# alebal123bal/BayesOpt_smart

Measured on AMD Instinct MI355X. Metric: candidate-points/sec (GP predict + HVI) at N_train=512, N_cand=1M, higher is better.
Workload: dtype f64; 1 GPU; C3: 2D/2-obj toy_function, N_train=512, N_cand=1,048,576 per GPU ('ij' integer grid), HVI (Sigma-UCB), q=3; n_train=512, n_cand_per_gpu=1048576, n_cand_total=1048576, n_objectives=2, dim=2, topq=3, parallelism=candidate-shard x1, step_launch=hip_graph, candidate_offset=0

## Files before the change

bayesopt_smart_amd/csrc/bo_gridconv.hip:

```cpp

#include "bo_predict_impl.h"

namespace {

using namespace bo;

constexpr int kListWaves = 4;
constexpr int kListChunk = 512;
#ifndef BO_ACC_RB
#define BO_ACC_RB 8
#endif
constexpr int kAccRB = BO_ACC_RB;
constexpr int kAccRows = 64 * kAccRB;
constexpr int kAccUnroll = 4;
constexpr int kClassLists = kConvClasses * kConvShards;
static_assert(kClassLists % 64 == 0 && kClassLists <= 2 * 64 * kConvAccWaves &&
              (kConvShards & (kConvShards - 1)) == 0 && kConvShards <= 16 && kConvShards <= kConvCountStride,
              "conv_acc_kernel's scan and lookup of the class lists");
#ifndef BO_CONV_PF
#define BO_CONV_PF 3
#endif
constexpr int kConvPF = BO_CONV_PF;
constexpr int kContractWaves = 8;
constexpr size_t kConvLdsBytes = 160 * 1024;
constexpr double kPairDrop = 0x1p-100;
constexpr double kTabFlush = 0x1p-128;

struct ListLds {
  int order, rc, nm;
  size_t bytes;
  __host__ __device__ ListLds(int n, int C)
      : order(C + 1), rc(order + n), nm(rc + 2 * n), bytes((size_t)(nm + kListWaves * kListChunk) * sizeof(int)) {}
};
struct AccLds {
  int ints, part;
  size_t bytes;
  __host__ __device__ explicit AccLds(int R)
      : ints(4 * R), part(kClassLists + 1),
        bytes((size_t)ints * sizeof(double) + (size_t)(part + kConvAccWaves + 1) / 2 * 2 * sizeof(int)) {}
};
struct ContractLds {
  int HB, tabH, hband, cn;
  size_t bytes;
  __host__ __device__ ContractLds(int C, int Cpad, int LT, int NP, int lists = 0)
      : HB(Cpad + LT / 2), tabH(2 * HB), hband(tabH + Cpad + C - 1), cn(hband + 1),
        bytes((size_t)cn * sizeof(double) + (size_t)NP * sizeof(int)) {
    if (bytes < (size_t)lists * sizeof(TopEntry)) bytes = (size_t)lists * sizeof(TopEntry);
  }
};

__device__ __forceinline__ void conv_list_done(const ConvArgs& a, int tau, int kept, int lane, int dyn) {
  if (kept == 0) {
    for (int o = 0; o < a.n_obj; ++o) {
      double* row = a.T + ((size_t)o * a.LT + tau) * a.ldr;
      for (int i = lane; i < a.ldr; i += 64) row[i] = 0.0;
    }
  }
  if (lane == 0) {
    a.pkept[tau] = kept;
    if (dyn && kept > 0) {
      const int e = 31 - __clz(kept);
      const int cls = 2 * e + (e > 0 ? (kept >> (e - 1)) & 1 : 0);
      const int sh = tau & (kConvShards - 1);
      const int slot = atomicAdd(a.ccount + cls * kConvCountStride + sh, 1);
      a.clist[(size_t)(cls * kConvShards + sh) * (a.LT / kConvShards) + slot] = tau;
    }
  }
}

__global__ __launch_bounds__(64 * kListWaves) void conv_list_kernel(const ConvArgs a, int tau_blocks, int dyn) {
  if (__builtin_amdgcn_readfirstlane(*a.flag) != 0) return;
  const int tid = threadIdx.x;
  if ((int)blockIdx.x >= tau_blocks) {
    const long long total = (long long)a.NP * a.ldr;
    const long long stride = (long long)(gridDim.x - tau_blocks) * (64 * kListWaves);
    for (int o = 0; o < a.n_obj; ++o) {
      const double nhl = a.nhl[o], pv = a.pv[o];
      double* tm = a.Tm + (size_t)o * a.NP * a.ldr;
      for (long long t = (long long)(blockIdx.x - tau_blocks) * (64 * kListWaves) + tid; t < total; t += stride) {
        const int s = (int)(t / a.ldr), i = (int)(t - (long long)s * a.ldr);
        double v = 0.0;
        if (s < a.n && i < a.nrows) {
          const int n = a.order[s];
          const double d = (double)(a.row_lo + i - a.rc[2 * n]);
          v = pv * a.alpha[(size_t)o * a.n_pad + n] * exp(nhl * (d * d));
        }
        tm[t] = v;
      }
    }
    return;
  }
  extern __shared__ __attribute__((aligned(16))) int si[];
  const ListLds L(a.n, a.C);
  int* cstart = si;
  int* order = si + L.order;
  int* rc = si + L.rc;
  for (int t = tid; t <= a.C; t += 64 * kListWaves) cstart[t] = a.cstart[t];
  for (int t = tid; t < a.n; t += 64 * kListWaves) order[t] = a.order[t];
  for (int t = tid; t < 2 * a.n; t += 64 * kListWaves) rc[t] = a.rc[t];
  __syncthreads();
  const int lane = tid & 63, wave = tid >> 6;
  int* nm = si + L.nm + wave * kListChunk;
  const int tau = blockIdx.x * kListWaves + wave;
  if (tau >= a.LT) return;
  int s0 = 0, s1 = 0;
  for (int c = lane; c < a.C; c += 64) {
    const int h = cstart[c + 1] - cstart[c];
    const int x0 = tau - c, x1 = x0 + 1;
    s0 += h * cstart[x0 < 0 ? 0 : x0 > a.C ? a.C : x0];
    s1 += h * cstart[x1 < 0 ? 0 : x1 > a.C ? a.C : x1];
  }
#pragma unroll
  for (int d = 32; d > 0; d >>= 1) {
    s0 += __shfl_xor(s0, d, 64);
    s1 += __shfl_xor(s1, d, 64);
  }
  const int h0 = (tau + 1) >> 1, h1 = (tau + 2) >> 1;
  const int p0 = __builtin_amdgcn_readfirstlane((s0 + cstart[h0 > a.C ? a.C : h0]) >> 1);
  const int total = __builtin_amdgcn_readfirstlane((s1 + cstart[h1 > a.C ? a.C : h1]) >> 1) - p0;
  if (lane == 0) a.pstart[tau] = p0;
  if (total == 0) {
    conv_list_done(a, tau, 0, lane, dyn);
    return;
  }
  const int R2 = 2 * a.R;
  const int per = (a.n + 63) / 64;
  const int n_lo = lane * per < a.n ? lane * per : a.n;
  const int n_hi = n_lo + per < a.n ? n_lo + per : a.n;
  int mine = 0;
  for (int n = n_lo; n < n_hi; ++n) {
    const int pc = tau - rc[2 * n + 1];
    if (pc < 0 || pc >= a.C) continue;
    for (int s = cstart[pc]; s < cstart[pc + 1]; ++s) mine += order[s] >= n ? 1 : 0;
  }
  int incl = mine;
#pragma unroll
  for (int d = 1; d < 64; d <<= 1) {
    const int v = __shfl_up(incl, d, 64);
    if (lane >= d) incl += v;
  }
  const int first = incl - mine;
  int kept = 0;
  for (int cb = 0; cb < total; cb += kListChunk) {
    const int cnt = total - cb < kListChunk ? total - cb : kListChunk;
    if (first < cb + cnt && first + mine > cb) {
// ... 69 lines not shown
    const double* e = tb + s;
#pragma unroll
    for (int k = 0; k < kAccRB; ++k) ev[k] = e[it[k]];
  };
  auto term = [&](double wv, const double (&ev)[kAccRB]) {
#pragma unroll
    for (int k = 0; k < kAccRB; ++k) {
      const double t = __dmul_rn(wv, ev[k]);
      const double te = __builtin_fma(wv, ev[k], -t);
      const double s2 = __dadd_rn(hi[k], t);
      const double bb = __dsub_rn(s2, hi[k]);
      const double se = __dadd_rn(__dsub_rn(hi[k], __dsub_rn(s2, bb)), __dsub_rn(t, bb));
      hi[k] = s2;
      lo[k] = __dadd_rn(lo[k], __dadd_rn(se, te));
    }
  };
  int p = 0;
  for (; p + kAccUnroll <= cnt; p += kAccUnroll) {
    double wv[kAccUnroll];
    int sv[kAccUnroll];
#pragma unroll
    for (int u = 0; u < kAccUnroll; ++u) {
      wv[u] = w[p + u];
      sv[u] = sl[p + u];
    }
    double ev[2][kAccRB];
    gather(sv[0], ev[0]);
#pragma unroll
    for (int u = 0; u < kAccUnroll; ++u) {
      if (u + 1 < kAccUnroll) gather(sv[u + 1], ev[(u + 1) & 1]);
      term(wv[u], ev[u & 1]);
    }
  }
  for (; p < cnt; ++p) {
    double ev[kAccRB];
    gather(sl[p], ev);
    term(w[p], ev);
  }
#pragma unroll
  for (int k = 0; k < kAccRB; ++k) {
    const int i = ib + lane + 64 * k;
    if (FULL) Trow[i] = hi[k] + lo[k];
    else if (i < ldr) Trow[i] = i < nrows ? hi[k] + lo[k] : 0.0;
  }
}

__global__ __launch_bounds__(64 * kConvAccWaves) void conv_acc_kernel(
    const ConvArgs a, const double* __restrict__ pair_w, const int* __restrict__ pair_sl,
    const int* __restrict__ pstart, const int* __restrict__ pkept, const int* __restrict__ ccount,
    const int* __restrict__ clist, int* __restrict__ ticket, double* __restrict__ T, int nrb, int ngrp, int dyn) {
  if (__builtin_amdgcn_readfirstlane(*a.flag) != 0) return;
  extern __shared__ __attribute__((aligned(16))) double sd[];
  const int tid = threadIdx.x, lane = tid & 63, o = blockIdx.y;
  const double nhl = a.nhl[o];
  const int R2 = 2 * a.R;
  const AccLds L(a.R);
  double* tabE = sd;
  int* cst = (int*)(sd + L.ints);
  int* part = cst + L.part;
  for (int t = tid; t < 2 * R2; t += 64 * kConvAccWaves) {
    const int par = t >= R2 ? 1 : 0, h = t - par * R2;
    const double m = (double)(2 * h + par - (R2 - 2));
    tabE[t] = exp(0.5 * nhl * (m * m));
  }
  if (dyn) {
    int c[2], sum = 0;
#pragma unroll
    for (int u = 0; u < 2; ++u) {
      const int j = 2 * tid + u;
      c[u] = j < kClassLists ? ccount[(kConvClasses - 1 - j / kConvShards) * kConvCountStride + j % kConvShards] : 0;
      sum += c[u];
    }
    int incl = sum;
#pragma unroll
    for (int d = 1; d < 64; d <<= 1) {
      const int v = __shfl_up(incl, d, 64);
      if (lane >= d) incl += v;
    }
    if (lane == 63) part[tid >> 6] = incl;
    __syncthreads();
    int run = incl - sum;
    for (int w = 0; w < (tid >> 6); ++w) run += part[w];
#pragma unroll
    for (int u = 0; u < 2; ++u) {
      const int j = 2 * tid + u;
      if (j < kClassLists) cst[j] = run;
      run += c[u];
      if (j == kClassLists - 1) cst[kClassLists] = run;
    }
  }
  __syncthreads();
  const int n_items = (dyn ? cst[kClassLists] : a.LT) * nrb;
  const double* wo = pair_w + (size_t)o * a.n_pairs;
  const int g = blockIdx.x % ngrp;
  int* tk = ticket + (o * kConvTicketGroups + g) * kConvTicketStride;
  for (int k = (blockIdx.x / ngrp) * kConvAccWaves + (tid >> 6);;) {
    const int t = k * ngrp + g;
    if (t >= n_items) break;
    int nx = 0;
    if (dyn && lane == 0) nx = atomicAdd(tk, 1);
    const int oi = t / nrb, rb = t - oi * nrb;
    int tau = oi;
    if (dyn) {
      constexpr int per = kClassLists / 64;
      const unsigned long long b1 = __ballot(cst[per * lane + per] > oi);
      const int l1 = __builtin_ctzll(b1);
      const unsigned long long b2 = __ballot(cst[per * l1 + (lane < per ? lane : per - 1) + 1] > oi);
      const int j = per * l1 + __builtin_ctzll(b2);
      const int cls = kConvClasses - 1 - j / kConvShards;
      const int* list = clist + (size_t)(cls * kConvShards + j % kConvShards) * (a.LT / kConvShards);
      tau = __builtin_amdgcn_readfirstlane(list[oi - cst[j]]);
    }
    const int p0 = __builtin_amdgcn_readfirstlane(pstart[tau]);
    const int cnt = __builtin_amdgcn_readfirstlane(pkept[tau]);
    if (!dyn && cnt == 0) break;
    const int ib = rb * kAccRows;
    double* Trow = T + ((size_t)o * a.LT + tau) * a.ldr;
// ... 17 lines not shown

template <int NB, class BGen>
__device__ __forceinline__ void conv_gemm(const double* __restrict__ X, int ldr, int nkb, int g, d4 (&acc)[NB],
                                          BGen&& bgen) {
  double ring[kConvPF][4];
#pragma unroll
  for (int p = 0; p < kConvPF; ++p) conv_load_a(X, ldr, p < nkb ? p : nkb - 1, g, ring[p]);
  for (int kb0 = 0; kb0 < nkb; kb0 += kConvPF) {
#pragma unroll
    for (int p = 0; p < kConvPF; ++p) {
      const int kb = kb0 + p;
      if (kb < nkb) {
        double av[4];
#pragma unroll
        for (int s = 0; s < 4; ++s) av[s] = ring[p][s];
        const int nx = kb + kConvPF;
        conv_load_a(X, ldr, nx < nkb ? nx : nkb - 1, g, ring[p]);
        double bv[4][NB];
        bgen(kb, bv);
#pragma unroll
        for (int s = 0; s < 4; ++s)
#pragma unroll
          for (int nb = 0; nb < NB; ++nb) acc[nb] = mfma64(av[s], bv[s][nb], acc[nb]);
      }
    }
  }
}

template <int NB>
__global__ __launch_bounds__(64 * kContractWaves) void conv_contract_kernel(const ConvArgs a) {
  if (__builtin_amdgcn_readfirstlane(*a.flag) != 0) return;
  extern __shared__ __attribute__((aligned(16))) double sd[];
  const ContractLds L(a.C, a.Cpad, a.LT, a.NP);
  double* tabB = sd;
  double* tabH = sd + L.tabH;
  int* hband = (int*)(sd + L.hband);
  int* cn = (int*)(sd + L.cn);
  constexpr int TW = 16 * NB;
  const int tid = threadIdx.x, lane = tid & 63, wave = tid >> 6;
  const int nt = blockDim.x, W = nt >> 6;
  const int g = lane >> 4, jl = lane & 15;
  const int cb_n = a.Cpad / TW;
  const long long n_wt = (long long)(a.ldr / 16) * cb_n;
  const long long gi_lo = a.cand_offset, gi_hi = a.cand_offset + a.n_cand;
#ifndef BO_ABL_CT_NOOUT
  const bool outs = true;
#else
  const bool outs = a.ld_out < 0;
#endif
  for (int t = tid; t < a.NP; t += nt) cn[t] = t < a.n ? a.rc[2 * a.order[t] + 1] : 0;

  double lv = -__builtin_inf();
  long long li = -1;
  double tab_nhl = __builtin_nan("");
  for (long long base = (long long)blockIdx.x * W; base < n_wt; base += (long long)gridDim.x * W) {
    const long long wt = base + wave;
    const bool active = wt < n_wt;
    const long long wtc = active ? wt : n_wt - 1;
    const int i0 = (int)(wtc / cb_n) * 16, j0 = (int)(wtc % cb_n) * TW;
    double acq[NB][4];
    for (int o = 0; o < a.n_obj; ++o) {
      const double nhl = a.nhl[o];
      if (!(nhl == tab_nhl)) {
        __syncthreads();
        int mq = 0;
        int mm = 0;
#ifndef BO_ABL_CT_NOTAB
        for (int t = tid; t < 2 * L.HB; t += nt) {
          const int par = t >= L.HB ? 1 : 0, h = t - par * L.HB;
          const int mi = 2 * h + par - (a.LT - 1);
          const double m = (double)mi;
          const double v = exp(0.5 * nhl * (m * m));
          const bool flush = v < kTabFlush;
          tabB[t] = flush ? 0.0 : v;
          if (!flush) mq = max(mq, abs(mi));
        }
        for (int t = tid; t < a.Cpad + a.C - 1; t += nt) {
          const int mi = t - (a.C - 1);
          const double m = (double)mi;
          const double v = exp(nhl * (m * m));
          const bool flush = v < kTabFlush;
          tabH[t] = flush ? 0.0 : v;
          if (!flush) mm = max(mm, abs(mi));
        }
#else
        mm = min((int)sqrt(128.0 * 0.6931471805599453 / -nhl), a.C - 1);
        mq = min((int)sqrt(256.0 * 0.6931471805599453 / -nhl), a.LT - 1);
#endif
        if (tid < 2) hband[tid] = 0;
        __syncthreads();
#pragma unroll
        for (int d = 32; d > 0; d >>= 1) {
          mq = max(mq, __shfl_xor(mq, d, 64));
          mm = max(mm, __shfl_xor(mm, d, 64));
        }
        if (lane == 0) {
          atomicMax(hband, mq);
          atomicMax(hband + 1, mm);
        }
        __syncthreads();
        tab_nhl = nhl;
      }
      int kq_lo = 0, kq_hi = a.LT / 16;
      if (!a.full) {
        const int hq = hband[0];
        const int t_hi = 2 * (j0 + TW - 1) + hq < a.LT - 1 ? 2 * (j0 + TW - 1) + hq : a.LT - 1;
        const int t_lo = 2 * j0 - hq > 0 ? (2 * j0 - hq < t_hi ? 2 * j0 - hq : t_hi) : 0;
        kq_lo = __builtin_amdgcn_readfirstlane(t_lo >> 4);
        kq_hi = __builtin_amdgcn_readfirstlane((t_hi >> 4) + 1);
      }
      d4 aq[NB], am[NB];
#pragma unroll
      for (int nb = 0; nb < NB; ++nb) {
        aq[nb] = (d4){0.0, 0.0, 0.0, 0.0};
        am[nb] = (d4){0.0, 0.0, 0.0, 0.0};
      }
      const double* Tq = a.T + ((size_t)o * a.LT + 16 * kq_lo) * a.ldr + i0 + jl;
      int km_lo = 0, km_hi = a.NP / 16;
      if (!a.full) {
        const int hm = hband[1];
        const int c_hi = j0 + TW + hm < a.C ? j0 + TW + hm : a.C;
        const int c_lo = j0 - hm > 0 ? (j0 - hm < a.C ? j0 - hm : a.C) : 0;
        km_lo = __builtin_amdgcn_readfirstlane(a.cstart[c_lo] >> 4);
        km_hi = __builtin_amdgcn_readfirstlane((a.cstart[c_hi] + 15) >> 4);
      }
      const double* Tm = a.Tm + ((size_t)o * a.NP + 16 * km_lo) * a.ldr + i0 + jl;
      const double* pe0 = tabB + (a.LT / 2 - 1 - 8 * kq_lo - 2 * g) + j0 + jl;
#ifdef BO_ABL_CT_BCONST
      const double bconst = pe0[0];
#endif
      conv_gemm<NB>(Tq, a.ldr, kq_hi - kq_lo, g, aq, [&](int kb, double (&bv)[4][NB]) {
#ifdef BO_ABL_CT_BCONST
#pragma unroll
        for (int s = 0; s < 4; ++s)
#pragma unroll
          for (int nb = 0; nb < NB; ++nb) bv[s][nb] = bconst;
#else
        const double* pe = pe0 - 8 * kb;
        const double* po = pe + L.HB;
#pragma unroll
        for (int nb = 0; nb < NB; ++nb) {
          bv[0][nb] = po[16 * nb];
          bv[1][nb] = pe[16 * nb];
          bv[2][nb] = po[16 * nb - 1];
          bv[3][nb] = pe[16 * nb - 1];
        }
#endif
      });
      const int* cn0 = cn + 16 * km_lo + 4 * g;
      if (km_hi > km_lo) conv_gemm<NB>(Tm, a.ldr, km_hi - km_lo, g, am, [&](int kb, double (&bv)[4][NB]) {
#ifdef BO_ABL_CT_BCONST
#pragma unroll
        for (int s = 0; s < 4; ++s)
#pragma unroll
// ... 161 lines not shown
      const long long e0 = (long long)gridDim.x * q, e1 = (long long)a.n_lists * q;
      for (long long e = e0 + tid; e < e1; e += nt) {
        a.partial[e].v = -__builtin_inf();
        a.partial[e].i = -1;
      }
    }
  }
}

}

namespace bo {

bool conv_lds_admits(int n, int R, int C, int Cpad, int LT, int NP) {
  const size_t bound = ((size_t)4 * R + 2048) * sizeof(double) + ((size_t)(C + 1) + 3 * (size_t)n + 2048) * sizeof(int);
  assert(ConvSetupLds(n, C, 256).bytes <= bound && ListLds(n, C).bytes <= bound && AccLds(R).bytes <= bound);
  return bound <= kConvLdsBytes && ContractLds(C, Cpad, LT, NP).bytes <= kConvLdsBytes;
}

template <class K>
static hipError_t conv_lds_attr(K k, size_t lds) {
  if (lds <= 64 * 1024) return hipSuccess;
  return hipFuncSetAttribute((const void*)k, hipFuncAttributeMaxDynamicSharedMemorySize, (int)lds);
}

ConvSched conv_acc_schedule(int R, int LT, int ldr, int n_obj, int cus) {
  ConvSched sc;
  sc.nrb = (ldr + kAccRows - 1) / kAccRows;
  const long long items = (long long)LT * sc.nrb;
  const size_t tab = (size_t)4 * R * sizeof(double);
  const int per_cu = (int)(kConvLdsBytes / tab < 4 ? kConvLdsBytes / tab : 4);
  long long wgs = (long long)(cus > 0 ? cus : 256) * per_cu / n_obj;
  if (wgs > (items + kConvAccWaves - 1) / kConvAccWaves) wgs = (items + kConvAccWaves - 1) / kConvAccWaves;
  if (wgs < 1) wgs = 1;
  sc.wgs = (int)wgs;
  sc.ngrp = (int)(wgs < kConvTicketGroups ? wgs : kConvTicketGroups);
  sc.dyn = (items <= wgs * kConvAccWaves && wgs % sc.ngrp == 0) ? 0 : 1;
  return sc;
}

hipError_t launch_gridconv(const ConvArgs& ca, const ConvPlan& cp, const ConvSched& sc, hipStream_t st) {
  const size_t l1 = ListLds(ca.n, ca.C).bytes, la = AccLds(ca.R).bytes;
  const size_t l2 = ContractLds(ca.C, ca.Cpad, ca.LT, ca.NP, cp.waves * ca.topq).bytes;
  if (l1 > kConvLdsBytes || la > kConvLdsBytes) return hipErrorInvalidValue;
  if (cp.waves < 1 || cp.waves > kContractWaves || cp.grid > ca.n_lists) return hipErrorInvalidValue;
  auto* contract = cp.nb == 4 ? conv_contract_kernel<4> : cp.nb == 2 ? conv_contract_kernel<2> : conv_contract_kernel<1>;
  hipError_t e;
  if ((e = conv_lds_attr(conv_list_kernel, l1)) != hipSuccess) return e;
  if ((e = conv_lds_attr(conv_acc_kernel, la)) != hipSuccess) return e;
  if ((e = conv_lds_attr(contract, l2)) != hipSuccess) return e;
  const int tau_blocks = (ca.LT + kListWaves - 1) / kListWaves;
  const long long tm_elems = (long long)ca.NP * ca.ldr;
  const int tm_blocks = (int)((tm_elems + 1023) / 1024 < 512 ? (tm_elems + 1023) / 1024 : 512);
  hipLaunchKernelGGL(conv_list_kernel, dim3(tau_blocks + tm_blocks), dim3(64 * kListWaves), l1, st, ca, tau_blocks,
                     sc.dyn);
  if ((e = hipGetLastError()) != hipSuccess) return e;
  hipLaunchKernelGGL(conv_acc_kernel, dim3((unsigned)sc.wgs, ca.n_obj), dim3(64 * kConvAccWaves), la, st, ca,
                     (const double*)ca.pair_w, (const int*)ca.pair_sl, (const int*)ca.pstart, (const int*)ca.pkept,
                     (const int*)ca.ccount, (const int*)ca.clist, ca.ticket, ca.T, sc.nrb, sc.ngrp, sc.dyn);
  if ((e = hipGetLastError()) != hipSuccess) return e;
  hipLaunchKernelGGL(contract, dim3(cp.grid), dim3(64 * cp.waves), l2, st, ca);
  return hipGetLastError();
}

}
```

bayesopt_smart_amd/csrc/bo_predict.hip:

```cpp

#include "bo_predict_impl.h"

#include <vector>

namespace {

__device__ __forceinline__ double kstar_at(const FusedArgs& a, int o, int f, long long j, bool valid) {
  return (valid && f < a.n_train) ? a.kstar[((long long)o * a.ks_rows + f) * a.n_cand + j] : 0.0;
}

template <int NS, bool SELECT>
__device__ __forceinline__ void contract_epair(__amdgpu_buffer_rsrc_t wr, int voff, int base,
                                               int& pos, int ep, const double (&B)[NS],
                                               d2 (&wa)[kPF], d2 (&wb)[kPF], d4& acc0, d4& acc1,
                                               double (&sel0)[4], double (&sel1)[4]) {
  constexpr int NCH = NS / 8;
#pragma unroll
  for (int c = 0; c < NCH; ++c) {
#pragma unroll
    for (int pp = 0; pp < 4; ++pp) {
      const int p = 4 * c + pp;
      const d2 ca = wa[pp];
      const d2 cb = wb[pp];
      const int so = base + ((pos + kPF) << 11);
// ... 400 lines not shown
  return cus;
}

constexpr double kConvMargin = 1.15;
constexpr int kConvMaxN = 4096;

void plan_gridconv(const bo_predict_desc* d, Plan* pl, bool kmem, int cus) {
  if (kmem || !pl->cm || d->cand_kind != BO_CAND_GRID || d->dim != 2 || d->n_cand <= 0) return;
  if (d->mode & (BO_PREDICT_DENSE | BO_PREDICT_NO_SEPARABLE | BO_PREDICT_FP32 | BO_PREDICT_NO_GRID_CONV)) return;
  const char* env = getenv("BO_GRID_CONV");
  if (env && env[0] == '0' && env[1] == 0) return;
  const long long R = d->grid_shape[0], C = d->grid_shape[1], n = d->n_train;
  if (R < 1 || C < 1 || R > (1 << 15) || C > (1 << 15) || n > kConvMaxN) return;
  if (d->cand_offset < 0 || d->cand_offset + d->n_cand > R * C) return;
  bo::ConvPlan cp = {};
  cp.row_lo = (int)(d->cand_offset / C);
  cp.nrows = (int)((d->cand_offset + d->n_cand - 1) / C) - cp.row_lo + 1;
  cp.ldr = (cp.nrows + 15) / 16 * 16;
  cp.Cpad = (int)((C + 63) / 64 * 64);
  cp.LT = (int)((2 * C - 1 + 15) / 16 * 16);
  cp.NP = (int)((n + 15) / 16 * 16);
  if (!bo::conv_lds_admits((int)n, (int)R, (int)C, cp.Cpad, cp.LT, cp.NP)) return;
  const long long wave_tiles = (long long)(cp.ldr / 16) * (cp.Cpad / 64);
  if (!(d->mode & (BO_PREDICT_GRID_CONV | BO_PREDICT_GRID_CONV_FULL))) {
    const double nch = pl->n_pad / 32;
    const double F = (double)d->n_obj * 1024.0 * nch * (nch + 1);
    const double old_rounds = (double)(((d->n_cand + 63) / 64 + 255) / 256);
    const double old_us = 25.0 + old_rounds * 64.0 * (F / 273.0e3 + 0.038);
    const double pairs_per_tau = 0.5 * (double)n * (double)(n + 1) / (double)(2 * C - 1);
    const double pair_us = 2.2 * pairs_per_tau * (double)((cp.ldr + 1023) / 1024) *
                           (double)((d->n_obj * (2 * C - 1) + 4095) / 4096);
    const double tile_rounds = (double)((wave_tiles + 1023) / 1024);
    const double contract_us = tile_rounds * 2048.0 * (double)(cp.LT + cp.NP) * (double)d->n_obj / 48.8e3;
    const double conv_us = 60.0 + pair_us + contract_us;
    if (!(kConvMargin * conv_us < old_us)) return;
  }
  cp.planned = true;
  const long long tiles64 = wave_tiles;
  cp.nb = tiles64 >= 8LL * cus ? 4 : 2 * tiles64 >= 8LL * cus ? 2 : 1;
  const char* tile = getenv("BO_CONV_TILE");
  if (tile && (tile[0] == '1' || tile[0] == '2' || tile[0] == '4') && tile[1] == 0) cp.nb = tile[0] - '0';
  const long long tiles = tiles64 * (4 / cp.nb);
  cp.waves = tiles >= 8LL * cus ? 8 : 4;
  long long wgs = (tiles + cp.waves - 1) / cp.waves;
#ifdef BO_ABL_CT_W4
  cp.waves = 4;
  wgs = (tiles + 3) / 4;
  if (wgs > 2LL * cus) wgs = 2LL * cus;
#else
  if (wgs > cus) wgs = cus;
#endif
  if (wgs > (long long)pl->grid * pl->waves) wgs = (long long)pl->grid * pl->waves;
  cp.grid = (int)wgs;
  cp.ws = bo::conv_layout(n, d->n_obj, C, cp.LT, cp.NP, cp.ldr, align256(pl->total));
  pl->total = cp.ws.end;
  pl->conv = cp;
}

int make_plan(const bo_predict_desc* d, Plan* pl, bool query_device, bool kmem = false) {
  if (!d || d->n_obj < 1 || d->n_obj > BO_MAX_OBJ || d->dim < 1 || d->dim > BO_MAX_DIM)
    return BO_ERR_ARG;
  if (d->n_train < 1 || d->n_cand < 0 || d->topq < 0 || d->topq > BO_MAX_TOPQ) return BO_ERR_ARG;
  if (d->cand_kind < 0 || d->cand_kind > BO_CAND_SOBOL) return BO_ERR_ARG;
  if (d->mode & ~(BO_PREDICT_DENSE | BO_PREDICT_NO_SEPARABLE | BO_PREDICT_FP32 | BO_PREDICT_F32_FLOOR |
                  BO_PREDICT_NO_GRID_CONV | BO_PREDICT_GRID_CONV | BO_PREDICT_GRID_CONV_FULL))
    return BO_ERR_ARG;
  if (d->excl_points && d->n_excl < 0) return BO_ERR_ARG;
  const long long n = d->n_train;
  if (n > (1 << 14)) return BO_ERR_UNSUPPORTED;
  memset(pl, 0, sizeof(*pl));
  pl->dim_pad = pad_dim(d->dim);
  pl->n_excl = (int)(d->excl_points ? d->n_excl : n);
  pl->n_panels = 1;
  if ((d->mode & BO_PREDICT_FP32) && !kmem) {
    const int n_pad = (int)((n + 63) / 64 * 64);
    const size_t lds = ((size_t)n_pad * pl->dim_pad + (size_t)d->n_obj * n_pad) * sizeof(float);
    if (lds <= kLdsBytes) {
      pl->fp32 = true;
      pl->n_pad = n_pad;
      pl->ns = 16;
      pl->lds = lds;
    }
  }
  if (!pl->fp32 && !kmem) {
    const int n_pad = pad_rows(n);
    const size_t base = (size_t)n_pad * pl->dim_pad + (size_t)d->n_obj * n_pad;
    pl->cm = true;
    pl->n_pad = n_pad;
    pl->ns = n_pad / 4;
    const size_t plain = base + bo::kExpTab;
    size_t lds = plain;
    if (d->cand_kind == BO_CAND_GRID && !(d->mode & BO_PREDICT_NO_SEPARABLE)) {
      const long long S = d->grid_shape[d->dim - 1];
      const size_t tbl = (size_t)d->n_obj * (2 * S - 1);
      const size_t rw_c = (size_t)n_pad * (d->n_obj + 1) + (size_t)(S + 63) / 64;
      const size_t lds_c = base + tbl + (size_t)kWaves * rw_c;
      const size_t lds_1 = base + tbl + (size_t)kWaves * n_pad * 2;
      if (S % 16 == 0 && S <= 32768 && d->cand_offset % 16 == 0 && lds_1 <= kLdsDoubles) {
        pl->sep = true;
        pl->rw_cache = lds_c <= kLdsDoubles;
        pl->rw_stride = (int)(pl->rw_cache ? rw_c : (size_t)n_pad * 2);
        pl->off_tbl = (int)base;
        pl->off_rw = (int)(base + tbl);
        lds = pl->rw_cache ? lds_c : lds_1;
        if (lds < plain) lds = plain;
      }
    }
// ... 185 lines not shown
  fa.off_rw = pl.off_rw;
  fa.rw_cache = pl.rw_cache ? 1 : 0;
  fa.rw_stride = pl.rw_stride;
  fa.off_exp = pl.off_exp;
  fa.conv_flag = pl.conv.planned ? (int*)(ws + pl.off_status + 32) : nullptr;
  return BO_OK;
}

static void fill_conv_args(const bo_predict_desc* d, const Plan& pl, char* ws, const FusedArgs& fa, bo::ConvArgs& ca) {
  const bo::ConvPlan& cp = pl.conv;
  const bo::ConvLayout& L = cp.ws;
  memset(&ca, 0, sizeof(ca));
  ca.n_obj = d->n_obj;
  ca.n = (int)d->n_train;
  ca.n_pad = pl.n_pad;
  ca.R = (int)d->grid_shape[0];
  ca.C = (int)d->grid_shape[1];
  ca.lo0 = d->grid_lo[0];
  ca.lo1 = d->grid_lo[1];
  ca.cand_offset = d->cand_offset;
  ca.n_cand = d->n_cand;
  ca.ld_out = fa.ld_out;
  ca.row_lo = cp.row_lo;
  ca.nrows = cp.nrows;
  ca.ldr = cp.ldr;
  ca.LT = cp.LT;
  ca.NP = cp.NP;
  ca.Cpad = cp.Cpad;
  ca.flag = (int*)fa.conv_flag;
  ca.x = d->x_train;
  ca.kinv = d->kinv;
  ca.ld_k = d->ld_k;
  ca.alpha = fa.alpha;
  memcpy(ca.pm, fa.pm, sizeof(ca.pm));
  memcpy(ca.pv, fa.pv, sizeof(ca.pv));
  memcpy(ca.nhl, fa.nhl, sizeof(ca.nhl));
  memcpy(ca.beta, fa.beta, sizeof(ca.beta));
  memcpy(ca.inv_rsq_pv, fa.inv_rsq_pv, sizeof(ca.inv_rsq_pv));
  memcpy(ca.inv_pv, fa.inv_pv, sizeof(ca.inv_pv));
  ca.min_var = fa.min_var;
  ca.cstart = (int*)(ws + L.cstart);
  ca.order = (int*)(ws + L.order);
  ca.rc = (int*)(ws + L.rc);
  ca.pstart = (int*)(ws + L.pstart);
  ca.pkept = (int*)(ws + L.pkept);
  ca.clist = (int*)(ws + L.clist);
  ca.ticket = (int*)(ws + L.ticket);
  ca.ccount = (int*)(ws + L.ccount);
  ca.Tm = (double*)(ws + L.Tm);
  ca.T = (double*)(ws + L.T);
  ca.pair_sl = (int*)(ws + L.pair_sl);
  ca.pair_w = (double*)(ws + L.pair_w);
  ca.n_pairs = (int)(d->n_train * (d->n_train + 1) / 2);
  ca.full = (d->mode & BO_PREDICT_GRID_CONV_FULL) ? 1 : 0;
  ca.mu = fa.mu;
  ca.var = fa.var;
  ca.std_mu = fa.std_mu;
  ca.std_var = fa.std_var;
  ca.ucb = fa.ucb;
  ca.acq = fa.acq;
  ca.topq = d->topq;
  ca.partial = fa.partial;
  ca.n_lists = pl.grid * pl.waves;
  ca.excl_pts = fa.excl ? fa.excl : fa.xpad;
  ca.hkeys = fa.hkeys;
  ca.hidx = fa.hidx;
  ca.hmask = fa.hmask;
}

static size_t fill_prep_args(const bo_predict_desc* d, const Plan& pl, char* ws, bool kmem, const FusedArgs& fa,
                             PrepArgs& pa) {
  memset(&pa, 0, sizeof(pa));
  pa.pack_mode = pl.fp32 ? 2 : (pl.cm ? 0 : 1);
  pa.wpack = ws;
  pa.kinv = d->kinv;
  pa.ld_k = d->ld_k;
  pa.upper = fa.upper;
  pa.n = (int)d->n_train;
  pa.n_pad = pl.n_pad;
  pa.ns = pl.ns;
  pa.n_obj = d->n_obj;
  const long long total = pl.fp32 ? c32_blocks(pl.n_pad / 64) * 1024 * d->n_obj
                        : pl.cm ? cm_blocks(pl.n_pad / 32, fa.upper) * 512 * d->n_obj
                                : (long long)d->n_obj * pl.n_pad * pl.n_pad / 2;
  pa.pack_blocks = (int)((total + 255) / 256 < 2048 ? (total + 255) / 256 : 2048);
  pa.alpha_blocks = (int)(((long long)d->n_obj * pl.n_pad + 3) / 4);
  pa.alpha = (double*)fa.alpha;
  pa.y = d->y_train;
  pa.ld_y = d->ld_y;
  for (int o = 0; o < d->n_obj; ++o) pa.pm[o] = d->prior_mean[o];
  pa.rows = kmem ? 0 : 1;
  pa.xpad = (double*)fa.xpad;
  pa.xc = (double*)fa.xc;
  pa.x = d->x_train;
  pa.dim = d->dim;
  pa.DIM = pl.dim_pad;
  pa.sep_flag = (int*)fa.sep_flag;
  pa.sep_lo = fa.sep_lo;
  pa.sep_S = fa.sep_S;
  pa.excl = (double*)(ws + pl.off_excl);
  pa.excl_in = d->excl_points;
  pa.n_excl = (kmem || !d->excl_points) ? 0 : pl.n_excl;
  pa.hkeys = (unsigned long long*)fa.hkeys;
  pa.hidx = (int*)fa.hidx;
  pa.hslots = pl.hash_slots;
  pa.n_hash = (kmem || d->topq == 0) ? 0 : pl.n_excl;
// ... 163 lines not shown
```

bayesopt_smart_amd/csrc/bo_predict_impl.h:

```cpp
#pragma once

#include "bo_common.h"

#include <assert.h>
#include <math.h>
#include <stdlib.h>
#include <string.h>

#include <type_traits>

namespace bo {

constexpr int kWaves = 4;
constexpr int kTile = 16 * kWaves;
constexpr int kPanelSteps = 128;
constexpr int kPF = 4;
constexpr int kCMaxEp = 16;
constexpr int kC32MaxEp = 16;
constexpr int kExpTab = 256;

struct FusedArgs {
  int n_obj, dim, n_train, n_pad;
  int n_panels;
  int n_excl;
// ... 11 lines not shown
  double pm[BO_MAX_OBJ], pv[BO_MAX_OBJ], nhl[BO_MAX_OBJ], beta[BO_MAX_OBJ];
  double inv_rsq_pv[BO_MAX_OBJ], inv_pv[BO_MAX_OBJ];
  double min_var;
  int idx32;
  double *mu, *var, *std_mu, *std_var, *ucb, *acq;
  TopEntry* partial;
  const double* kstar;
  long long ks_rows;
  int upper;
  const int* sep_flag;
  int sep_S;
  long long sep_lo;
  int off_tbl, off_rw;
  int rw_cache;
  int rw_stride;
  int off_exp;
  SobolArgs sob;
  const unsigned long long* hkeys;
  const int* hidx;
  unsigned int hmask;
  const int* conv_flag;
};

struct ConvArgs {
  int n_obj, n, n_pad;
  int R, C;
  long long lo0, lo1;
  long long cand_offset, n_cand, ld_out;
  int row_lo, nrows, ldr;
  int LT;
  int NP;
  int Cpad;
  int* flag;
  const double* x;
  const double* kinv;
  long long ld_k;
  const double* alpha;
  double pm[BO_MAX_OBJ], pv[BO_MAX_OBJ], nhl[BO_MAX_OBJ], beta[BO_MAX_OBJ];
  double inv_rsq_pv[BO_MAX_OBJ], inv_pv[BO_MAX_OBJ];
  double min_var;
  int* cstart;
  int* order;
  int* rc;
  int* pstart;
  int* pkept;
  int* ccount;
  int* clist;
  int* ticket;
  int n_pairs;
  int* pair_sl;
  double* pair_w;
  double* T;
  double* Tm;
  double *mu, *var, *std_mu, *std_var, *ucb, *acq;
  int topq;
  int full;
  TopEntry* partial;
  int n_lists;
  const double* excl_pts;
  const unsigned long long* hkeys;
  const int* hidx;
  unsigned int hmask;
};

constexpr int kConvTicketGroups = 32;
constexpr int kConvTicketStride = 32;
constexpr int kConvClasses = 64;
#ifndef BO_CONV_SHARDS
#define BO_CONV_SHARDS 8
#endif
constexpr int kConvShards = BO_CONV_SHARDS;
constexpr int kConvCountStride = 32;
constexpr int kConvAccWaves = 4;

struct ConvSched {
  int nrb;
  int wgs, ngrp;
  int dyn;
};

struct ConvSetupLds {
  int col, part;
  size_t bytes;
  __host__ __device__ ConvSetupLds(int n, int C, int threads)
      : col(C + 1), part(col + n), bytes((size_t)(part + threads / 64) * sizeof(int)) {}
};

template <int THREADS>
__device__ __forceinline__ void conv_scan(int* v, int len, int* part, int* out) {
  const int tid = threadIdx.x, lane = tid & 63, wave = tid >> 6;
  const int seg = (len + THREADS - 1) / THREADS;
  const int c_lo = tid * seg < len ? tid * seg : len, c_hi = c_lo + seg < len ? c_lo + seg : len;
  int sum = 0;
  for (int c = c_lo; c < c_hi; ++c) sum += v[c];
  int incl = sum;
#pragma unroll
  for (int d = 1; d < 64; d <<= 1) {
    const int t = __shfl_up(incl, d, 64);
    if (lane >= d) incl += t;
  }
  if (lane == 63) part[wave] = incl;
  __syncthreads();
  int run = incl - sum;
  for (int w = 0; w < wave; ++w) run += part[w];
  for (int c = c_lo; c < c_hi; ++c) {
    const int t = v[c];
// ... 8 lines not shown
__device__ __forceinline__ void conv_setup_block(const ConvArgs& a, const ConvSched& sc, int* lds) {
  const ConvSetupLds L(a.n, a.C, THREADS);
  int* cnt = lds;
  int* col = lds + L.col;
  int* part = lds + L.part;
  const int tid = threadIdx.x, lane = tid & 63;
  for (int c = tid; c <= a.C; c += THREADS) cnt[c] = 0;
  for (int t = tid; t < a.n_obj * sc.ngrp; t += THREADS) {
    const int g = t % sc.ngrp;
    a.ticket[(t / sc.ngrp * kConvTicketGroups + g) * kConvTicketStride] =
        (sc.wgs - g + sc.ngrp - 1) / sc.ngrp * kConvAccWaves;
  }
  for (int t = tid; t < kConvClasses * kConvShards; t += THREADS)
    a.ccount[t / kConvShards * kConvCountStride + t % kConvShards] = 0;
  __syncthreads();
  for (int n = tid; n < a.n; n += THREADS) {
    const int r = (int)fmin(fmax(a.x[2 * (long long)n] - (double)a.lo0, 0.0), (double)(a.R - 1));
    const int c = (int)fmin(fmax(a.x[2 * (long long)n + 1] - (double)a.lo1, 0.0), (double)(a.C - 1));
    a.rc[2 * n] = r;
    a.rc[2 * n + 1] = c;
    col[n] = c;
    atomicAdd(cnt + c, 1);
  }
  __syncthreads();
  conv_scan<THREADS>(cnt, a.C + 1, part, a.cstart);
  if (tid >= 64) return;
  const int bits = a.C > 1 ? 32 - __clz(a.C - 1) : 0;
  for (int n0 = 0; n0 < a.n; n0 += 64) {
    const int n = n0 + lane;
    const bool valid = n < a.n;
    const int c = valid ? col[n] : 0;
    unsigned long long m = __ballot(valid);
    for (int b = 0; b < bits; ++b) {
      const bool bit = (c >> b) & 1;
      const unsigned long long bal = __ballot(valid && bit);
      m &= bit ? bal : ~bal;
    }
    const unsigned long long below = m & ((1ull << lane) - 1ull);
    const int base = valid ? cnt[c] : 0;
    __builtin_amdgcn_fence(__ATOMIC_RELEASE, "wavefront");
    __builtin_amdgcn_wave_barrier();
    __builtin_amdgcn_fence(__ATOMIC_ACQUIRE, "wavefront");
    if (valid) {
      a.order[base + __popcll(below)] = n;
      if (below == 0ull) cnt[c] = base + __popcll(m);
    }
    __builtin_amdgcn_fence(__ATOMIC_RELEASE, "wavefront");
    __builtin_amdgcn_wave_barrier();
    __builtin_amdgcn_fence(__ATOMIC_ACQUIRE, "wavefront");
  }
}

struct ConvLayout {
  size_t cstart, order, rc, pstart, pkept, clist, ticket, ccount, Tm, T, pair_sl, pair_w, end;
};

inline ConvLayout conv_layout(long long n, int n_obj, long long C, long long LT, long long NP, long long ldr,
                              size_t base) {
  size_t at = base;
  auto take = [&at](long long count, size_t elem, size_t align) {
    const size_t off = (at + align - 1) / align * align;
    at = off + (size_t)count * elem;
    return off;
  };
  const long long pairs = n * (n + 1) / 2;
  ConvLayout L;
  L.cstart = take(C + 1, sizeof(int), 256);
  L.order = take(n, sizeof(int), sizeof(int));
  L.rc = take(2 * n, sizeof(int), sizeof(int));
  L.pstart = take(LT, sizeof(int), sizeof(int));
  L.pkept = take(LT, sizeof(int), sizeof(int));
  L.clist = take(kConvClasses * LT, sizeof(int), sizeof(int));
  L.ticket = take(BO_MAX_OBJ * kConvTicketGroups * kConvTicketStride, sizeof(int), 128);
  L.ccount = take(kConvClasses * kConvCountStride, sizeof(int), 128);
  L.Tm = take(n_obj * NP * ldr, sizeof(double), 256);
  L.T = take(n_obj * LT * ldr, sizeof(double), 256);
  L.pair_sl = take(pairs, sizeof(int), 256);
  L.pair_w = take(n_obj * pairs, sizeof(double), 256);
  L.end = take(0, 1, 256) + (L.ticket % 256 == 0 ? 256 : 0);
  return L;
}

bool conv_lds_admits(int n, int R, int C, int Cpad, int LT, int NP);
ConvSched conv_acc_schedule(int R, int LT, int ldr, int n_obj, int cus);

struct ConvPlan {
  bool planned;
  int nb;
  int waves;
  int grid;
  int row_lo, nrows, ldr, LT, NP, Cpad;
  ConvLayout ws;
};

hipError_t launch_gridconv(const ConvArgs& ca, const ConvPlan& cp, const ConvSched& sc, hipStream_t st);

struct Plan {
  int n_pad, ns, n_panels, dim_pad, n_excl;
  bool multi;
  size_t off_alpha, off_xpad, off_xc, off_excl, off_hash, off_partial, off_status, total;
  unsigned int hash_slots;
  bool cm;
  bool sep;
  bool grows;
  int off_tbl, off_rw;
  bool rw_cache;
  int rw_stride;
  bool fp32;
  bool small;
  int off_exp;
  int grid, waves;
  long long n_tiles;
  size_t lds;
  ConvPlan conv;
};

hipError_t launch_cm_d2(const Plan& pl, const FusedArgs& fa, hipStream_t st);
hipError_t launch_cm_d4(const Plan& pl, const FusedArgs& fa, hipStream_t st);
hipError_t launch_cm_d6(const Plan& pl, const FusedArgs& fa, hipStream_t st);
hipError_t launch_cm_d8(const Plan& pl, const FusedArgs& fa, hipStream_t st);
hipError_t launch_c32_d2(const Plan& pl, const FusedArgs& fa, hipStream_t st);
hipError_t launch_c32_d4(const Plan& pl, const FusedArgs& fa, hipStream_t st);
hipError_t launch_c32_d6(const Plan& pl, const FusedArgs& fa, hipStream_t st);
hipError_t launch_c32_d8(const Plan& pl, const FusedArgs& fa, hipStream_t st);
hipError_t launch_cms_d2(const Plan& pl, const FusedArgs& fa, hipStream_t st);
hipError_t launch_cms_d4(const Plan& pl, const FusedArgs& fa, hipStream_t st);
hipError_t launch_cms_d6(const Plan& pl, const FusedArgs& fa, hipStream_t st);
hipError_t launch_cms_d8(const Plan& pl, const FusedArgs& fa, hipStream_t st);

}

namespace {
// ... 986 lines not shown
```

Baseline: 5.408 billion candidate-points/sec.

## Precompute Gaussian exp tables once per objective in list kernel, copy into LDS

```diff
diff --git a/bayesopt_smart_amd/csrc/bo_gridconv.hip b/bayesopt_smart_amd/csrc/bo_gridconv.hip
--- a/bayesopt_smart_amd/csrc/bo_gridconv.hip
+++ b/bayesopt_smart_amd/csrc/bo_gridconv.hip
@@ -68,12 +68,71 @@
   }
 }
 
-__global__ __launch_bounds__(64 * kListWaves) void conv_list_kernel(const ConvArgs a, int tau_blocks, int dyn) {
+__device__ __forceinline__ void conv_table_block(const ConvArgs& a, int b, int* red) {
+  constexpr int NT = 64 * kListWaves;
+  const int tid = threadIdx.x;
+  const int o = b / 3, which = b - 3 * o;
+  if (a.tab_of[o] != o) return;
+  const double nhl = a.nhl[o];
+  int mx = 0;
+  if (which == 0) {
+    const int R2 = 2 * a.R;
+    double* tab = a.tabE + (size_t)o * 2 * R2;
+    for (int t = tid; t < 2 * R2; t += NT) {
+      const int par = t >= R2 ? 1 : 0, h = t - par * R2;
+      const int mi = 2 * h + par - (R2 - 2);
+      const double m = (double)mi;
+      const double v = exp(0.5 * nhl * (m * m));
+      const bool flush = v < kTabFlush;
+      tab[t] = flush ? 0.0 : v;
+      if (!flush) mx = max(mx, abs(mi));
+    }
+  } else if (which == 1) {
+    const int HB = ContractLds(a.C, a.Cpad, a.LT, a.NP).HB;
+    double* tab = a.tabB + (size_t)o * 2 * HB;
+    for (int t = tid; t < 2 * HB; t += NT) {
+      const int par = t >= HB ? 1 : 0, h = t - par * HB;
+      const int mi = 2 * h + par - (a.LT - 1);
+      const double m = (double)mi;
+      const double v = exp(0.5 * nhl * (m * m));
+      const bool flush = v < kTabFlush;
+      tab[t] = flush ? 0.0 : v;
+      if (!flush) mx = max(mx, abs(mi));
+    }
+  } else {
+    const int len = a.Cpad + a.C - 1;
+    double* tab = a.tabH + (size_t)o * len;
+    for (int t = tid; t < len; t += NT) {
+      const int mi = t - (a.C - 1);
+      const double m = (double)mi;
+      const double v = exp(nhl * (m * m));
+      const bool flush = v < kTabFlush;
+      tab[t] = flush ? 0.0 : v;
+      if (!flush) mx = max(mx, abs(mi));
+    }
+  }
+#pragma unroll
+  for (int d = 32; d > 0; d >>= 1) mx = max(mx, __shfl_xor(mx, d, 64));
+  if ((tid & 63) == 0) red[tid >> 6] = mx;
+  __syncthreads();
+  if (tid == 0) {
+    for (int w = 1; w < kListWaves; ++w) mx = max(mx, red[w]);
+    a.band[4 * o + which] = mx;
+  }
+}
+
+__global__ __launch_bounds__(64 * kListWaves) void conv_list_kernel(const ConvArgs a, int tau_blocks, int tm_blocks,
+                                                                    int dyn) {
   if (__builtin_amdgcn_readfirstlane(*a.flag) != 0) return;
+  extern __shared__ __attribute__((aligned(16))) int si[];
   const int tid = threadIdx.x;
+  if ((int)blockIdx.x >= tau_blocks + tm_blocks) {
+    conv_table_block(a, (int)blockIdx.x - tau_blocks - tm_blocks, si);
+    return;
+  }
   if ((int)blockIdx.x >= tau_blocks) {
     const long long total = (long long)a.NP * a.ldr;
-    const long long stride = (long long)(gridDim.x - tau_blocks) * (64 * kListWaves);
+    const long long stride = (long long)tm_blocks * (64 * kListWaves);
     for (int o = 0; o < a.n_obj; ++o) {
       const double nhl = a.nhl[o], pv = a.pv[o];
       double* tm = a.Tm + (size_t)o * a.NP * a.ldr;
@@ -90,7 +149,6 @@
     }
     return;
   }
-  extern __shared__ __attribute__((aligned(16))) int si[];
   const ListLds L(a.n, a.C);
   int* cstart = si;
   int* order = si + L.order;
@@ -266,17 +324,13 @@
   if (__builtin_amdgcn_readfirstlane(*a.flag) != 0) return;
   extern __shared__ __attribute__((aligned(16))) double sd[];
   const int tid = threadIdx.x, lane = tid & 63, o = blockIdx.y;
-  const double nhl = a.nhl[o];
   const int R2 = 2 * a.R;
   const AccLds L(a.R);
   double* tabE = sd;
   int* cst = (int*)(sd + L.ints);
   int* part = cst + L.part;
-  for (int t = tid; t < 2 * R2; t += 64 * kConvAccWaves) {
-    const int par = t >= R2 ? 1 : 0, h = t - par * R2;
-    const double m = (double)(2 * h + par - (R2 - 2));
-    tabE[t] = exp(0.5 * nhl * (m * m));
-  }
+  const double2* tsrc = (const double2*)(a.tabE + (size_t)a.tab_of[o] * 2 * R2);
+  for (int t = tid; t < R2; t += 64 * kConvAccWaves) ((double2*)tabE)[t] = tsrc[t];
   if (dyn) {
     int c[2], sum = 0;
 #pragma unroll
@@ -400,7 +454,7 @@
 
   double lv = -__builtin_inf();
   long long li = -1;
-  double tab_nhl = __builtin_nan("");
+  int tab_set = -1;
   for (long long base = (long long)blockIdx.x * W; base < n_wt; base += (long long)gridDim.x * W) {
     const long long wt = base + wave;
     const bool active = wt < n_wt;
@@ -408,46 +462,17 @@
     const int i0 = (int)(wtc / cb_n) * 16, j0 = (int)(wtc % cb_n) * TW;
     double acq[NB][4];
     for (int o = 0; o < a.n_obj; ++o) {
-      const double nhl = a.nhl[o];
-      if (!(nhl == tab_nhl)) {
+      const int ts = a.tab_of[o];
+      if (__builtin_expect(ts != tab_set, 0)) {
         __syncthreads();
-        int mq = 0;
-        int mm = 0;
-#ifndef BO_ABL_CT_NOTAB
-        for (int t = tid; t < 2 * L.HB; t += nt) {
-          const int par = t >= L.HB ? 1 : 0, h = t - par * L.HB;
-          const int mi = 2 * h + par - (a.LT - 1);
-          const double m = (double)mi;
-          const double v = exp(0.5 * nhl * (m * m));
-          const bool flush = v < kTabFlush;
-          tabB[t] = flush ? 0.0 : v;
-          if (!flush) mq = max(mq, abs(mi));
-        }
-        for (int t = tid; t < a.Cpad + a.C - 1; t += nt) {
-          const int mi = t - (a.C - 1);
-          const double m = (double)mi;
-          const double v = exp(nhl * (m * m));
-          const bool flush = v < kTabFlush;
-          tabH[t] = flush ? 0.0 : v;
-          if (!flush) mm = max(mm, abs(mi));
-        }
-#else
-        mm = min((int)sqrt(128.0 * 0.6931471805599453 / -nhl), a.C - 1);
-        mq = min((int)sqrt(256.0 * 0.6931471805599453 / -nhl), a.LT - 1);
-#endif
-        if (tid < 2) hband[tid] = 0;
+        const int lenH = a.Cpad + a.C - 1;
+        const double* sB = a.tabB + (size_t)ts * 2 * L.HB;
+        const double* sH = a.tabH + (size_t)ts * lenH;
+        for (int t = tid; t < 2 * L.HB; t += nt) tabB[t] = sB[t];
+        for (int t = tid; t < lenH; t += nt) tabH[t] = sH[t];
+        if (tid < 2) hband[tid] = a.band[4 * ts + 1 + tid];
         __syncthreads();
-#pragma unroll
-        for (int d = 32; d > 0; d >>= 1) {
-          mq = max(mq, __shfl_xor(mq, d, 64));
-          mm = max(mm, __shfl_xor(mm, d, 64));
-        }
-        if (lane == 0) {
-          atomicMax(hband, mq);
-          atomicMax(hband + 1, mm);
-        }
-        __syncthreads();
-        tab_nhl = nhl;
+        tab_set = ts;
       }
       int kq_lo = 0, kq_hi = a.LT / 16;
       if (!a.full) {
@@ -715,8 +740,8 @@
   const int tau_blocks = (ca.LT + kListWaves - 1) / kListWaves;
   const long long tm_elems = (long long)ca.NP * ca.ldr;
   const int tm_blocks = (int)((tm_elems + 1023) / 1024 < 512 ? (tm_elems + 1023) / 1024 : 512);
-  hipLaunchKernelGGL(conv_list_kernel, dim3(tau_blocks + tm_blocks), dim3(64 * kListWaves), l1, st, ca, tau_blocks,
-                     sc.dyn);
+  hipLaunchKernelGGL(conv_list_kernel, dim3(tau_blocks + tm_blocks + 3 * ca.n_obj), dim3(64 * kListWaves), l1, st, ca,
+                     tau_blocks, tm_blocks, sc.dyn);
   if ((e = hipGetLastError()) != hipSuccess) return e;
   hipLaunchKernelGGL(conv_acc_kernel, dim3((unsigned)sc.wgs, ca.n_obj), dim3(64 * kConvAccWaves), la, st, ca,
                      (const double*)ca.pair_w, (const int*)ca.pair_sl, (const int*)ca.pstart, (const int*)ca.pkept,
diff --git a/bayesopt_smart_amd/csrc/bo_predict.hip b/bayesopt_smart_amd/csrc/bo_predict.hip
--- a/bayesopt_smart_amd/csrc/bo_predict.hip
+++ b/bayesopt_smart_amd/csrc/bo_predict.hip
@@ -476,7 +476,7 @@
 #endif
   if (wgs > (long long)pl->grid * pl->waves) wgs = (long long)pl->grid * pl->waves;
   cp.grid = (int)wgs;
-  cp.ws = bo::conv_layout(n, d->n_obj, C, cp.LT, cp.NP, cp.ldr, align256(pl->total));
+  cp.ws = bo::conv_layout(n, d->n_obj, R, C, cp.Cpad, cp.LT, cp.NP, cp.ldr, align256(pl->total));
   pl->total = cp.ws.end;
   pl->conv = cp;
 }
@@ -768,6 +768,18 @@
   ca.pair_sl = (int*)(ws + L.pair_sl);
   ca.pair_w = (double*)(ws + L.pair_w);
   ca.n_pairs = (int)(d->n_train * (d->n_train + 1) / 2);
+  ca.tabE = (double*)(ws + L.tabE);
+  ca.tabB = (double*)(ws + L.tabB);
+  ca.tabH = (double*)(ws + L.tabH);
+  ca.band = (int*)(ws + L.band);
+  for (int o = 0; o < d->n_obj; ++o) {
+    ca.tab_of[o] = o;
+    for (int p = 0; p < o; ++p)
+      if (fa.nhl[p] == fa.nhl[o]) {
+        ca.tab_of[o] = p;
+        break;
+      }
+  }
   ca.full = (d->mode & BO_PREDICT_GRID_CONV_FULL) ? 1 : 0;
   ca.mu = fa.mu;
   ca.var = fa.var;
diff --git a/bayesopt_smart_amd/csrc/bo_predict_impl.h b/bayesopt_smart_amd/csrc/bo_predict_impl.h
--- a/bayesopt_smart_amd/csrc/bo_predict_impl.h
+++ b/bayesopt_smart_amd/csrc/bo_predict_impl.h
@@ -87,6 +87,11 @@
   double* pair_w;
   double* T;
   double* Tm;
+  int tab_of[BO_MAX_OBJ];
+  double* tabE;
+  double* tabB;
+  double* tabH;
+  int* band;
   double *mu, *var, *std_mu, *std_var, *ucb, *acq;
   int topq;
   int full;
@@ -201,11 +206,11 @@
 }
 
 struct ConvLayout {
-  size_t cstart, order, rc, pstart, pkept, clist, ticket, ccount, Tm, T, pair_sl, pair_w, end;
+  size_t cstart, order, rc, pstart, pkept, clist, ticket, ccount, Tm, T, pair_sl, pair_w, tabE, tabB, tabH, band, end;
 };
 
-inline ConvLayout conv_layout(long long n, int n_obj, long long C, long long LT, long long NP, long long ldr,
-                              size_t base) {
+inline ConvLayout conv_layout(long long n, int n_obj, long long R, long long C, long long Cpad, long long LT,
+                              long long NP, long long ldr, size_t base) {
   size_t at = base;
   auto take = [&at](long long count, size_t elem, size_t align) {
     const size_t off = (at + align - 1) / align * align;
@@ -226,7 +231,12 @@
   L.T = take(n_obj * LT * ldr, sizeof(double), 256);
   L.pair_sl = take(pairs, sizeof(int), 256);
   L.pair_w = take(n_obj * pairs, sizeof(double), 256);
-  L.end = take(0, 1, 256) + (L.ticket % 256 == 0 ? 256 : 0);
+  at = take(0, 1, 256) + (L.ticket % 256 == 0 ? 256 : 0);
+  L.tabE = take(n_obj * 4 * R, sizeof(double), 256);
+  L.tabB = take(n_obj * 2 * (Cpad + LT / 2), sizeof(double), 256);
+  L.tabH = take(n_obj * (Cpad + C - 1), sizeof(double), 256);
+  L.band = take(n_obj * 4, sizeof(int), 256);
+  L.end = take(0, 1, 256);
   return L;
 }
 
```

After: 5.441 billion candidate-points/sec, median of 3. Within noise of the previous version (+0.6%).
